# arnauqb/GradABM-JUNE

Measured on NVIDIA B200. Metric: agent_timesteps_per_sec_fwd_bwd, higher is better.
Workload: dtype f32

## Files before the change

### gradabm-june_b200/csrc/gj_kernels.cu

```cuda
#include <cuda_runtime.h>
#include <math.h>
#include <stdint.h>
#include <stdio.h>
#include <stdlib.h>
#include <string.h>

#include "gj_device.cuh"
#include "gj_tiled.cuh"
#include "gj_lean.cuh"
#include "gj_pipe.cuh"

namespace gj {

static thread_local char g_err[512] = "";

static int fail(const char* what, cudaError_t e) {
  snprintf(g_err, sizeof(g_err), "%s: %s", what, cudaGetErrorString(e));
  return -2;
}
static int bad(const char* what) {
  snprintf(g_err, sizeof(g_err), "invalid argument: %s", what);
  return -1;
}
#define GJ_CHECK_LAUNCH(name)                         \
// ... 743 lines not shown
  if (w->n_small > 0 || w->n_chunks > 0) {
    ProfScope ps(bwd ? K_GROUP_CHUNK_B : K_GROUP_CHUNK_F, st);
    const int chunk_blocks = w->n_chunks > 0 ? blocks_for(w->n_chunks * 32, kBlock) : 0;
    const int small_blocks = w->n_small > 0 ? blocks_for(w->n_small, kBlock) : 0;
    launch_pdl(k_lean_group_sums, dim3((chunk_blocks + small_blocks) * bt.nb), dim3(kBlock), 0, st, *w, *p, pl, beta, in,
               out_scaled, out_plain, sc.part_a, chunk_blocks, bt);
    GJ_CHECK_LAUNCH("k_lean_group_sums");
  }
  if (w->n_big > 0) {
    ProfScope ps(bwd ? K_GROUP_FIX_B : K_GROUP_FIX_F, st);
    launch_pdl(k_lean_group_fix, dim3(blocks_for(w->n_big * 32, kBlock) * bt.nb), dim3(kBlock), 0, st, *w, *p, pl, beta,
               (const float*)sc.part_a, out_scaled, out_plain, bt);
    GJ_CHECK_LAUNCH("k_lean_group_fix");
  }
  return 0;
}

static int lean_forward(const gj_world_desc* w, const gj_step_params* p, const Plan& pl, const LeanPlan& lp,
                        const gj_fwd_io* io, const Scratch& sc, cudaStream_t st, const NextStep* next,
                        const Batch& bt = kNoBatch) {
  const bool quar = p->n_quar > 0;
  const bool batch = bt.nb > 1;
  if (p->stage != GJ_STAGE_REST) {
    if (!p->t_ready) {
      ProfScope ps(K_TRANSMISSION, st);
      static OccCache occ[4];
      const Scatter sct{sc.sct_acc, sc.sct_dirty};
#define GJ_K1(Q, B, I)                                                                                               \
  launch_pdl(k_lean_transmission<Q, B>, dim3(lean_grid(w, k_lean_transmission<Q, B>, &occ[I], bt)), dim3(kLeanThreads), \
             0, st, *w, *p, lp, *io, sc.tile_part, sct, bt)
#define GJ_K1C(Q, B, I)                                                                                              \
  launch_pdl(k_lean_transmission_c<Q, B>, dim3(lean_grid(w, k_lean_transmission_c<Q, B>, &occ_c[I], bt)),              \
             dim3(kLeanThreads), 0, st, *w, *p, lp, *io, sc.tile_part, sct, bt)
      static OccCache occ_c[4];
      const bool compact = (pipe_flags() & 4) == 0;
      if (compact) {
        if (batch) {
          if (quar) GJ_K1C(true, true, 3);
          else GJ_K1C(false, true, 2);
        } else {
          if (quar) GJ_K1C(true, false, 1);
          else GJ_K1C(false, false, 0);
        }
      } else if (batch) {
        if (quar) GJ_K1(true, true, 3);
        else GJ_K1(false, true, 2);
      } else {
        if (quar) GJ_K1(true, false, 1);
        else GJ_K1(false, false, 0);
      }
#undef GJ_K1
#undef GJ_K1C
      GJ_CHECK_LAUNCH("k_lean_transmission");
    }
    if (lp.has_generic)
      if (int e = launch_lean_forward_sums(w, p, pl, io->beta, quar ? io->Tq : io->T, io->S_scaled + lp.gen_base,
                                           io->S_unscaled + lp.gen_base, sc, st, bt))
        return e;
    if (int e = launch_cell_groups(w, p, pl, io->beta, io->S_scaled, io->S_unscaled, sc, st, bt)) return e;
  }
  if (p->stage == GJ_STAGE_SUMS) return 0;
  if (int e = launch_cell_gather(w, p, pl, io->S_scaled, sc, st, bt)) return e;
  if (batch && bt.noise && pipe_enabled() && pipe_aligned_fwd(w, lp, io)) {
    ProfScope pn(K_OTHER, st);
    launch_pdl(k_batch_noise, dim3(agent_grid(w->n_agents)), dim3(kBlock), 0, st, *w, *p, const_cast<float*>(bt.noise));
    GJ_CHECK_LAUNCH("k_batch_noise");
  }
  if (pipe_enabled() && pipe_aligned_fwd(w, lp, io)) {
    ProfScope ps(K_AGENT_FWD, st);
    static OccCache occ[20];
    const bool diag = io->q || io->n;
    const bool lab = io->label != nullptr;
    const size_t smem = next ? sizeof(PipeFwdSharedT<true, false>)
                             : (batch ? sizeof(PipeFwdSharedT<false, true>) : sizeof(PipeFwdSharedT<false, false>));
    NextStep nx;
    memset(&nx, 0, sizeof(nx));
    if (next) {
      nx = *next;
      nx.tile_part = sc.tile_part;
      nx.sct = Scatter{sc.sct_acc, sc.sct_dirty};
    }
#define GJ_PIPE_FWD(Q, D, X, B, L, I)                                                                                 \
  launch_pdl(k_pipe_forward<Q, D, X, B, L>,                                                                           \
             dim3(pipe_grid(w, k_pipe_forward<Q, D, X, B, L>, kPipeThreads, smem, &occ[I], bt)), dim3(kPipeThreads),    \
             smem, st, *w, *p, lp, *io, (const float*)sc.cell_buf, sc.red_part, sc.tickets, nx, bt)
    if (lab && batch) {
      if (quar && diag) GJ_PIPE_FWD(true, true, false, true, true, 19);
      else if (quar) GJ_PIPE_FWD(true, false, false, true, true, 18);
      else if (diag) GJ_PIPE_FWD(false, true, false, true, true, 17);
      else GJ_PIPE_FWD(false, false, false, true, true, 16);
    } else if (lab) {
      if (quar && diag) GJ_PIPE_FWD(true, true, false, false, true, 15);
      else if (quar) GJ_PIPE_FWD(true, false, false, false, true, 14);
      else if (diag) GJ_PIPE_FWD(false, true, false, false, true, 13);
      else GJ_PIPE_FWD(false, false, false, false, true, 12);
    } else if (batch) {
      if (quar && diag) GJ_PIPE_FWD(true, true, false, true, false, 11);
      else if (quar) GJ_PIPE_FWD(true, false, false, true, false, 10);
      else if (diag) GJ_PIPE_FWD(false, true, false, true, false, 9);
      else GJ_PIPE_FWD(false, false, false, true, false, 8);
    } else if (next) {
      if (quar && diag) GJ_PIPE_FWD(true, true, true, false, false, 7);
      else if (quar) GJ_PIPE_FWD(true, false, true, false, false, 6);
      else if (diag) GJ_PIPE_FWD(false, true, true, false, false, 5);
      else GJ_PIPE_FWD(false, false, true, false, false, 4);
    } else {
      if (quar && diag) GJ_PIPE_FWD(true, true, false, false, false, 3);
      else if (quar) GJ_PIPE_FWD(true, false, false, false, false, 2);
      else if (diag) GJ_PIPE_FWD(false, true, false, false, false, 1);
      else GJ_PIPE_FWD(false, false, false, false, false, 0);
    }
#undef GJ_PIPE_FWD
    GJ_CHECK_LAUNCH("k_pipe_forward");
    return next ? 1 : 0;
  }
  if (batch) return bad("batched step: the pipelined kernels are off or an array is not 16-byte aligned");
  {
    ProfScope ps(K_AGENT_FWD, st);
    static OccCache occ[8];
    const bool diag = io->q || io->n;
#define GJ_LEAN_FWD(Q, D, L, I)                                                                                       \
  k_lean_forward<Q, D, L><<<lean_grid(w, k_lean_forward<Q, D, L>, &occ[I]), kLeanThreads, 0, st>>>(                   \
      *w, *p, lp, *io, sc.cell_buf, sc.red_part, sc.tickets)
    if (io->label) {
      if (quar && diag) GJ_LEAN_FWD(true, true, true, 7);
      else if (quar) GJ_LEAN_FWD(true, false, true, 6);
      else if (diag) GJ_LEAN_FWD(false, true, true, 5);
      else GJ_LEAN_FWD(false, false, true, 4);
    } else {
      if (quar && diag) GJ_LEAN_FWD(true, true, false, 3);
      else if (quar) GJ_LEAN_FWD(true, false, false, 2);
      else if (diag) GJ_LEAN_FWD(false, true, false, 1);
      else GJ_LEAN_FWD(false, false, false, 0);
    }
#undef GJ_LEAN_FWD
    GJ_CHECK_LAUNCH("k_lean_forward");
  }
  return 0;
}

static int lean_backward(const gj_world_desc* w, const gj_step_params* p, const Plan& pl, LeanPlan lp,
                         const gj_bwd_io* io, const Scratch& sc, cudaStream_t st, const Batch& bt = kNoBatch) {
  const bool quar = p->n_quar > 0;
  const bool batch = bt.nb > 1;
  static OccCache occ_b[4], occ_g[2];
  const bool lab = io->label && io->g_red_label;
  int gather_grid = 1;
  const bool pipe = pipe_enabled() && pipe_aligned_bwd(w, lp, io);
  if (batch && !pipe) return bad("batched step: the pipelined kernels are off or an array is not 16-byte aligned");
  if (p->stage != GJ_STAGE_REST) {
    if (pipe) {
      ProfScope ps(K_AGENT_BWD, st);
      static OccCache occ[8];
      const size_t smem = sizeof(PipeBwdShared);
#define GJ_PIPE_BWD(Q, B, L, I)                                                                                       \
  launch_pdl(k_pipe_backward<Q, B, L>, dim3(pipe_grid(w, k_pipe_backward<Q, B, L>, kBwdThreads, smem, &occ[I], bt)),    \
             dim3(kBwdThreads), smem, st, *w, *p, lp, *io, sc.tile_part, bt)
      if (lab && batch) {
        if (quar) GJ_PIPE_BWD(true, true, true, 7);
        else GJ_PIPE_BWD(false, true, true, 6);
      } else if (lab) {
        if (quar) GJ_PIPE_BWD(true, false, true, 5);
        else GJ_PIPE_BWD(false, false, true, 4);
      } else if (batch) {
        if (quar) GJ_PIPE_BWD(true, true, false, 3);
        else GJ_PIPE_BWD(false, true, false, 2);
      } else {
// ... 767 lines not shown
```

### gradabm-june_b200/csrc/gj_lean.cuh

```cuda
#pragma once
#include "gj_tiled.cuh"

namespace gj {

constexpr int kLeanThreads = 256;
#ifndef GJ_LEAN_MINB_FWD
#define GJ_LEAN_MINB_FWD 3
#endif
#ifndef GJ_LEAN_MINB_BWD
#define GJ_LEAN_MINB_BWD 4
#endif
#ifndef GJ_LEAN_MINB_GATHER
#define GJ_LEAN_MINB_GATHER 3
#endif
constexpr uint32_t kEntNone = 0xFFFFFFFFu;
constexpr uint32_t kEntMulti = 0xFFFFFFFEu;
constexpr uint32_t kEntGiant = 0x80000000u;
constexpr uint32_t kEntId = 0x7FFFFFFFu;

struct Scatter {
  unsigned long long* acc;
  uint8_t* dirty;
};
constexpr float kScatterScale = (float)(1ull << GJ_SCATTER_FRAC);
// ... 57 lines not shown
  const float sg = d + 1e-10f;
  const float sign01 = (sg > 0.0f) ? 1.0f : ((sg == 0.0f) ? 0.5f : 0.0f);
  const float x = d * pf.y;
  const float pe = ex2_fast(fmaf(pf.z, lg2_fast(x), -x * 1.4426950408889634f));
  TransTerms r;
  r.coef = (pf.x * sign01) * pe;
  r.dcoef = 0.0f;
  if (kGrad) r.dcoef = r.coef * pf.y * (1.0f - pf.z * rcp_fast(x));
  return r;
}

__global__ void __launch_bounds__(kBlock) k_profile_pack(int64_t n, const float* __restrict__ maxinf,
                                                         const float* __restrict__ shape,
                                                         const float* __restrict__ rate,
                                                         const float* __restrict__ shift, const float* __restrict__ k0,
                                                         float4* __restrict__ out) {
  const int64_t stride = (int64_t)gridDim.x * blockDim.x;
  for (int64_t a = (int64_t)blockIdx.x * blockDim.x + threadIdx.x; a < n; a += stride)
    out[a] = make_float4((maxinf[a] * k0[a]) * rate[a], rate[a], shape[a] - 1.0f, shift[a]);
}

struct TileRun {
  int64_t t0, t1;
};
__device__ __forceinline__ TileRun lean_tiles(const gj_world_desc& w) {
  TileRun r;
  r.t0 = w.n_tiles * (int64_t)blockIdx.x / gridDim.x;
  r.t1 = w.n_tiles * ((int64_t)blockIdx.x + 1) / gridDim.x;
  return r;
}
__device__ __forceinline__ TileRun lean_tiles(const gj_world_desc& w, const BatchCta& bc) {
  TileRun r;
  r.t0 = w.n_tiles * (int64_t)bc.bx / bc.gx;
  r.t1 = w.n_tiles * ((int64_t)bc.bx + 1) / bc.gx;
  return r;
}
__device__ __forceinline__ int64_t lean_segment_end(const LeanPlan& lp, int64_t tile, int64_t t1) {
  int64_t e = t1;
  for (int i = 0; i < lp.n_tc; ++i) {
    const int64_t c = lp.ctp[i][lp.tc[i][tile] + 1];
    e = c < e ? c : e;
  }
  return e;
}
__device__ __forceinline__ bool lean_new_cell(const LeanPlan& lp, int64_t a, int64_t b) {
  bool changed = false;
  for (int i = 0; i < lp.n_tc; ++i) changed = changed || (lp.tc[i][a] != lp.tc[i][b]);
  return changed;
}

struct alignas(16) ProbRow {
  float v[GJ_MAX_CHANNELS];
};
template <bool kCareSide>
__device__ __forceinline__ void lean_load_prob(ProbRow* prob, const gj_step_params& p, const LeanPlan& lp,
                                               const float* __restrict__ lprob) {
  for (int i = threadIdx.x; i < GJ_MAX_CHANNELS * 200; i += blockDim.x) {
    const int j = i / 200, c = i - j * 200;
    float v = 0.0f;
    if (j < lp.n_cell) {
      v = lprob[(size_t)(lp.c_row[j] * 2 + p.day_type) * 200 + c];
      if (kCareSide && lp.c_care[j] && age_of(c) <= 75) v = 0.0f;
    }
    prob[c].v[j] = v;
  }
}

__device__ __forceinline__ void lean_channel_fma(float (&acc)[GJ_MAX_CHANNELS], const ProbRow* prob, int cls, float x,
                                                 int n_cell) {
  const float4 lo = *reinterpret_cast<const float4*>(&prob[cls].v[0]);
  acc[0] = fmaf(lo.x, x, acc[0]);
  acc[1] = fmaf(lo.y, x, acc[1]);
  acc[2] = fmaf(lo.z, x, acc[2]);
  acc[3] = fmaf(lo.w, x, acc[3]);
  if (n_cell > 4) {
    const float4 hi = *reinterpret_cast<const float4*>(&prob[cls].v[4]);
    acc[4] = fmaf(hi.x, x, acc[4]);
    acc[5] = fmaf(hi.y, x, acc[5]);
    acc[6] = fmaf(hi.z, x, acc[6]);
    acc[7] = fmaf(hi.w, x, acc[7]);
  }
}

__device__ __forceinline__ void lean_class_table(float* __restrict__ L, const ProbRow* prob, const LeanPlan& lp,
                                                 const float* __restrict__ cell_buf, int64_t tile) {
  const int lane = threadIdx.x & 31;
  float mine = 0.0f;
  if (lane < lp.n_cell)
    mine = cell_buf[(lp.c_cell_off[lane] + lp.c_tile_cell[lane][tile]) * GJ_MAX_CHANNELS + lane];
  float acc = 0.0f;
  const int c = threadIdx.x < 200 ? threadIdx.x : 0;
#pragma unroll
  for (int j = 0; j < GJ_MAX_CHANNELS; ++j) {
    const float v = __shfl_sync(0xffffffffu, mine, j);
    acc = fmaf(v, prob[c].v[j], acc);
  }
  if (threadIdx.x < 200) L[threadIdx.x] = acc;
}

__device__ __forceinline__ float lean_generic_issue(const float* __restrict__ buf, uint32_t ent) {
  return (ent < kEntMulti) ? buf[ent & kEntId] : 0.0f;
}
__device__ __forceinline__ float lean_generic_finish(const gj_world_desc& w, const float* __restrict__ buf, uint32_t ent,
                                                     uint32_t a, float v) {
  if (ent == kEntMulti) {
    for (uint32_t j = w.am_ptr[a]; j < w.am_ptr[a + 1]; ++j) {
      const uint32_t e = w.am_ent[j];
      v += buf[w.type_group_off[e >> 28] + (e & 0x0FFFFFFFu)];
    }
  }
  return v;
}

struct RangeLoads {
  float x[8];
};
__device__ __forceinline__ RangeLoads lean_range_issue(const float* __restrict__ v, uint32_t a, uint32_t slot) {
  RangeLoads r;
  const uint32_t b0 = a - (slot >> 16);
  const int nb = (slot == kNoSlot) ? 0 : (int)(slot & 0xFFFFu);
#pragma unroll
  for (int j = 0; j < 8; ++j) r.x[j] = (j < nb) ? v[b0 + j] : 0.0f;
  return r;
}
__device__ __forceinline__ float lean_range_finish(const RangeLoads& r, const float* __restrict__ v, uint32_t a,
                                                   uint32_t slot) {
  float S = ((r.x[0] + r.x[1]) + (r.x[2] + r.x[3])) + ((r.x[4] + r.x[5]) + (r.x[6] + r.x[7]));
  if (slot != kNoSlot && (slot & 0xFFFFu) > 8u) {
    const uint32_t b0 = a - (slot >> 16), nb = slot & 0xFFFFu;
    for (uint32_t b = b0 + 8; b < b0 + nb; ++b) S += v[b];
  }
  return S;
}

__device__ __forceinline__ float quar_mask(const gj_step_params& p, float cur) {
  bool ok = true;
#pragma unroll
  for (int i = 0; i < GJ_MAX_QUAR; ++i)
    if (i < p.n_quar) ok = ok && (cur < p.quar_thr[i]);
  return ok ? 1.0f : 0.0f;
}

#ifndef GJ_K1_BATCH
#define GJ_K1_BATCH 2
#endif
#ifndef GJ_K1_MINB
#define GJ_K1_MINB 7
#endif
constexpr int kK1Batch = GJ_K1_BATCH;

template <bool kQuar, bool kBatch>
__global__ void __launch_bounds__(kLeanThreads, GJ_K1_MINB) k_lean_transmission(gj_world_desc w, gj_step_params p, LeanPlan lp,
                                                                    gj_fwd_io io, float* __restrict__ tile_part,
                                                                    Scatter sct, Batch bt) {
  __shared__ ProbRow prob[200];
  pdl_launch();
  lean_load_prob<false>(prob, p, lp, io.leisure_prob);
  pdl_wait();
  __syncthreads();
  const BatchCta bc = batch_cta<kBatch>(bt);
  const uint32_t so = bc.so;
  if (kBatch) {
    tile_part = scr_shift(tile_part, bt, bc.s);
    sct.acc = scr_shift(sct.acc, bt, bc.s);
    sct.dirty = scr_shift(sct.dirty, bt, bc.s);
  }
  const float4* __restrict__ prof = reinterpret_cast<const float4*>(io.prof4);
  const float* __restrict__ g_inf = io.inf;
  const float* __restrict__ g_cur = io.cur;
  const TileRun run = lean_tiles(w, bc);
  for (int64_t tile = run.t0; tile < run.t1;) {
    const int64_t tend = lp.n_cell > 0 ? lean_segment_end(lp, tile, run.t1) : run.t1;
    const uint32_t a0 = w.tile_begin[tile], a1 = w.tile_begin[tend];
    float acc[GJ_MAX_CHANNELS];
#pragma unroll
    for (int j = 0; j < GJ_MAX_CHANNELS; ++j) acc[j] = 0.0f;
    for (uint32_t base = a0 + threadIdx.x; base < a1; base += kK1Batch * kLeanThreads) {
      float inf[kK1Batch], cur[kK1Batch];
#pragma unroll
// ... 897 lines not shown
```

### gradabm-june_b200/csrc/gj_pipe.cuh

```cuda
#pragma once
#include "gj_lean.cuh"

namespace gj {

constexpr int kPipeThreads = 512;
constexpr int kPipeTile = GJ_TILE_AGENTS;
constexpr int kPipeHalo = 64;
constexpr int kPipeStages = 2;
constexpr int kPipeWarps = kPipeThreads / 32;
constexpr int kPipePer = kPipeTile / kPipeThreads;
static_assert(kPipePer * kPipeThreads == kPipeTile, "tile = whole agents per thread");

__device__ __forceinline__ uint32_t smem_u32(const void* p) { return (uint32_t)__cvta_generic_to_shared(p); }
__device__ __forceinline__ void mbar_init(uint64_t* bar, uint32_t count) {
  asm volatile("mbarrier.init.shared::cta.b64 [%0], %1;" ::"r"(smem_u32(bar)), "r"(count));
}
__device__ __forceinline__ void mbar_expect_tx(uint64_t* bar, uint32_t bytes) {
  asm volatile("mbarrier.arrive.expect_tx.shared::cta.b64 _, [%0], %1;" ::"r"(smem_u32(bar)), "r"(bytes) : "memory");
}
__device__ __forceinline__ void mbar_wait(uint64_t* bar, uint32_t parity) {
  asm volatile(
      "{\n"
      ".reg .pred p;\n"
      "WAIT_%=:\n"
      "mbarrier.try_wait.parity.shared::cta.b64 p, [%0], %1;\n"
      "@p bra DONE_%=;\n"
      "bra WAIT_%=;\n"
      "DONE_%=:\n"
      "}\n" ::"r"(smem_u32(bar)),
      "r"(parity)
      : "memory");
}
__device__ __forceinline__ void bulk_g2s(void* dst, const void* src, uint32_t bytes, uint64_t* bar) {
  asm volatile("cp.async.bulk.shared::cluster.global.mbarrier::complete_tx::bytes [%0], [%1], %2, [%3];" ::"r"(
                   smem_u32(dst)),
               "l"(src), "r"(bytes), "r"(smem_u32(bar))
               : "memory");
}

struct TileSpan {
  uint32_t a0, a1, lo4, hi4, n4;
  uint32_t tlo, thi;
  uint32_t lo16, hi16;
};
__device__ __forceinline__ TileSpan tile_span(const gj_world_desc& w, int64_t tile) {
  TileSpan t;
  t.a0 = w.tile_begin[tile];
  t.a1 = w.tile_begin[tile + 1];
  t.lo4 = t.a0 & ~3u;
  t.hi4 = (t.a1 + 3u) & ~3u;
  t.n4 = (t.hi4 - t.lo4) * 4u;
  const uint32_t nmax = (uint32_t)((w.n_agents + 3) & ~(int64_t)3);
  t.tlo = (t.a0 > (uint32_t)kPipeHalo ? t.a0 - kPipeHalo : 0u) & ~3u;
  t.thi = (t.a1 + kPipeHalo + 3u) & ~3u;
  if (t.thi > nmax) t.thi = nmax;
  t.lo16 = t.a0 & ~15u;
  t.hi16 = (t.a1 + 15u) & ~15u;
  return t;
}
__device__ __forceinline__ uint32_t halo_lo(uint32_t a0) { return (a0 > (uint32_t)kPipeHalo ? a0 - kPipeHalo : 0u) & ~3u; }

struct Copier {
  uint64_t* bar;
  __device__ __forceinline__ void f4(void* dst, const void* base, const TileSpan& t) const {
    bulk_g2s(dst, reinterpret_cast<const char*>(base) + (size_t)t.lo4 * 4u, t.n4, bar);
  }
};

__device__ __forceinline__ float pipe_range_sum(const float* __restrict__ Ts, uint32_t tlo, uint32_t a, uint32_t slot) {
  if (slot == kNoSlot) return 0.0f;
  const uint32_t b0 = a - (slot >> 16) - tlo;
  const int nb = (int)(slot & 0xFFFFu);
  float x[8];
#pragma unroll
  for (int j = 0; j < 8; ++j) x[j] = (j < nb) ? Ts[b0 + j] : 0.0f;
  float S = ((x[0] + x[1]) + (x[2] + x[3])) + ((x[4] + x[5]) + (x[6] + x[7]));
  for (int j = 8; j < nb; ++j) S += Ts[b0 + j];
  return S;
}

struct TileWalk {
  uint32_t a1;
  uint32_t nxt_a1;
  uint32_t nxt_flag;
};
__device__ __forceinline__ TileWalk tile_walk_begin(const gj_world_desc& w, const LeanPlan& lp, const TileRun& run) {
  TileWalk t;
  t.a1 = t.nxt_a1 = 0;
  t.nxt_flag = 1u;
  if (run.t0 < run.t1) {
    t.a1 = w.tile_begin[run.t0];
    t.nxt_a1 = w.tile_begin[run.t0 + 1];
  }
  return t;
}
#define PIPE_TILE_FACTS                                                   \
  const uint32_t a0 = tw.a1, a1 = tw.nxt_a1;                              \
  const bool new_cell = lp.n_cell > 0 && (tw.nxt_flag & 1u);              \
  (void)new_cell;                                                         \
  tw.a1 = a1;                                                             \
  tw.nxt_flag = w.tile_flags[tile + 1];                                   \
  tw.nxt_a1 = w.tile_begin[tile + 2]
#define PIPE_FLUSH(tw, lp) ((lp).n_cell > 0 && (tile + 1 == run.t1 || ((tw).nxt_flag & 1u)))

__device__ __forceinline__ bool pipe_release() {
  __syncthreads();
  return threadIdx.x == 0;
}

constexpr int kPcLut = kPipeHalo + 8;
__device__ __forceinline__ void pipe_fill_pc_lut(float* lut) {
  for (int n = threadIdx.x; n < kPcLut; n += blockDim.x) lut[n] = fmaxf(fminf(1.0f / (float)(n - 1), 1.0f), 0.0f);
}

constexpr int kPipeF = kPipeTile + 8;
constexpr int kPipeH = kPipeTile + 2 * kPipeHalo + 8;

__device__ __forceinline__ void pipe_init_barriers(uint64_t* full) {
  if (threadIdx.x == 0) {
    for (int i = 0; i < kPipeStages; ++i) mbar_init(&full[i], 1);
    asm volatile("fence.mbarrier_init.release.cluster;" ::: "memory");
  }
}

struct NextStep {
  int on;
  float now;
  int day_type;
  int n_quar;
  float quar_thr[GJ_MAX_QUAR];
  int n_cell;
  int c_row[GJ_MAX_CHANNELS];
  int n_tc;
  const uint32_t* tc[GJ_MAX_CHANNELS];
  float* T;
  float* Tq;
  float* tile_part;
  int has_generic;
  Scatter sct;
};
__device__ __forceinline__ float quar_mask_next(const NextStep& nx, float cur) {
  bool ok = true;
#pragma unroll
  for (int i = 0; i < GJ_MAX_QUAR; ++i)
    if (i < nx.n_quar) ok = ok && (cur < nx.quar_thr[i]);
  return ok ? 1.0f : 0.0f;
}
__device__ __forceinline__ bool next_new_cell(const NextStep& nx, int64_t a, int64_t b) {
  bool changed = false;
  for (int i = 0; i < nx.n_tc; ++i) changed = changed || (nx.tc[i][a] != nx.tc[i][b]);
  return changed;
}
template <bool kBatch>
struct alignas(16) PipeFwdStageT {
  float s[kPipeF], inf[kPipeF], tinf[kPipeF], cur[kPipeF], nxt[kPipeF], ttn[kPipeF], rpc[kPipeF];
  uint32_t ent[kPipeF], slot[kPipeF], oid[kPipeF];
  float T[kPipeH];
  uint8_t cls[kPipeTile + 32];
  float dE[kBatch ? kPipeF : 4];
};
template <bool kNext, bool kBatch>
struct PipeFwdSharedT {
  PipeFwdStageT<kBatch> st[kPipeStages];
  ProbRow prob[200];
  ProbRow prob_next[kNext ? 200 : 1];
  float L[2][200];
  float beta[GJ_MAX_NETS];
  float hist[100];
  float deaths;
  float pc_lut[kPcLut];
  alignas(8) uint64_t full[kPipeStages];
};

template <bool kBatch>
__device__ __forceinline__ void pipe_fwd_issue(PipeFwdStageT<kBatch>& sg, uint64_t* bar, const gj_world_desc& w,
                                               const LeanPlan& lp, const gj_fwd_io& io, const float* Tr, int64_t tile,
                                               bool has_gen, bool has_range, uint32_t so = 0u,
                                               const float* noise = nullptr) {
  const TileSpan t = tile_span(w, tile);
  uint32_t total = 6u * t.n4 + (t.hi16 - t.lo16);
  if (kBatch && noise) total += t.n4;
  if (has_gen) total += t.n4;
  if (w.orig_id) total += t.n4;
  if (has_range) total += (lp.r_pc_lut ? 1u : 2u) * t.n4 + (t.thi - t.tlo) * 4u;
  mbar_expect_tx(bar, total);
  const Copier c{bar};
  if (kBatch && noise) c.f4(sg.dE, noise, t);
  if (w.orig_id) c.f4(sg.oid, w.orig_id, t);
  c.f4(sg.s, io.s + so, t);
  c.f4(sg.inf, io.inf + so, t);
  c.f4(sg.tinf, io.tinf + so, t);
  c.f4(sg.cur, io.cur + so, t);
  c.f4(sg.nxt, io.nxt + so, t);
  c.f4(sg.ttn, io.ttn + so, t);
  if (has_gen) c.f4(sg.ent, w.ent1, t);
  if (has_range) {
    c.f4(sg.slot, lp.r_slot, t);
    if (!lp.r_pc_lut) c.f4(sg.rpc, lp.r_pc, t);
    bulk_g2s(sg.T, Tr + so + t.tlo, (t.thi - t.tlo) * 4u, bar);
  }
  bulk_g2s(sg.cls, w.cls + t.lo16, t.hi16 - t.lo16, bar);
}

template <bool kQuar, bool kDiag, bool kNext, bool kBatch, bool kLabel>
__global__ void __launch_bounds__(kPipeThreads, 2) k_pipe_forward(gj_world_desc w, gj_step_params p, LeanPlan lp,
                                                                 gj_fwd_io io, const float* __restrict__ cell_buf,
                                                                 double* __restrict__ red_part,
                                                                 unsigned int* __restrict__ ticket, NextStep nx,
                                                                 Batch bt) {
  static_assert(!(kNext && kBatch), "the look-ahead transmission pass is not batched");
  static_assert(!(kNext && kLabel), "a step with a label table runs without the look-ahead");
  extern __shared__ __align__(128) unsigned char pipe_smem[];
  PipeFwdSharedT<kNext, kBatch>& sh = *reinterpret_cast<PipeFwdSharedT<kNext, kBatch>*>(pipe_smem);
  const BatchCta bc = batch_cta<kBatch>(bt);
  const float* noise = kBatch ? bt.noise : nullptr;
  const uint32_t so = bc.so;
  float* __restrict__ red_out = io.red;
  const float* __restrict__ beta_in = io.beta;
  uint32_t* __restrict__ lacc = io.label_acc;
  if (kBatch) {
    cell_buf = scr_shift(cell_buf, bt, bc.s);
    red_part = scr_shift(red_part, bt, bc.s);
    ticket = scr_shift(ticket, bt, bc.s);
    if (red_out) red_out += (int64_t)bc.s * bt.sRed;
    if (kLabel) lacc += bc.s * bt.sLab;
    beta_in += (int64_t)bc.s * bt.sBeta;
  }
  const TileRun run = lean_tiles(w, bc);
  const float* __restrict__ Tr = (kQuar && !lp.r_house) ? io.Tq : io.T;
  const bool has_gen = lp.has_generic != 0, has_range = lp.n_range > 0;
  pdl_launch();
  pipe_init_barriers(sh.full);
  lean_load_prob<true>(sh.prob, p, lp, io.leisure_prob);
  pipe_fill_pc_lut(sh.pc_lut);
  if (kNext) {
    for (int i = threadIdx.x; i < GJ_MAX_CHANNELS * 200; i += blockDim.x) {
      const int j = i / 200, c = i - j * 200;
      sh.prob_next[c].v[j] = j < nx.n_cell ? io.leisure_prob[(size_t)(nx.c_row[j] * 2 + nx.day_type) * 200 + c] : 0.0f;
    }
  }
  pdl_wait();
  if (threadIdx.x < p.n_nets) sh.beta[threadIdx.x] = beta_in[threadIdx.x];
  if (threadIdx.x < 100) sh.hist[threadIdx.x] = 0.0f;
  if (threadIdx.x == 0) sh.deaths = 0.0f;
  __syncthreads();
  if (threadIdx.x == 0) {
    for (int i = 0; i < kPipeStages; ++i)
      if (run.t0 + i < run.t1)
        pipe_fwd_issue<kBatch>(sh.st[i], &sh.full[i], w, lp, io, Tr, run.t0 + i, has_gen, has_range, so, noise);
  }
  const float* __restrict__ SP = io.S_scaled + lp.gen_base + (kBatch ? (int64_t)bc.s * bt.sG : (int64_t)0);
  const float dead = (float)(p.n_stages - 1);
  const float inv_tau = 1.0f / p.tau;
  const float beta_r = lp.n_range > 0 ? sh.beta[lp.r_net] : 0.0f;

  const float4* __restrict__ prof = reinterpret_cast<const float4*>(io.prof4);
  float acc[GJ_MAX_CHANNELS];
#pragma unroll
  for (int j = 0; j < GJ_MAX_CHANNELS; ++j) acc[j] = 0.0f;
  int nbuild = 0, stg = 0;
  uint32_t parity = 0;
  const float* L = sh.L[0];
  TileWalk tw = tile_walk_begin(w, lp, run);
  for (int64_t tile = run.t0; tile < run.t1; ++tile) {
    PipeFwdStageT<kBatch>& sg = sh.st[stg];
    PIPE_TILE_FACTS;
    mbar_wait(&sh.full[stg], parity);
    if (new_cell) {
      lean_class_table(sh.L[nbuild & 1], sh.prob, lp, cell_buf, tile);
      L = sh.L[nbuild & 1];
      ++nbuild;
      __syncthreads();
    }
    const uint32_t sk = a0 & 3u, sk16 = a0 & 15u, tlo = halo_lo(a0);
    uint32_t ent[kPipePer];
    float gen[kPipePer];
    float4 pfe[kPipePer];
#pragma unroll
    for (int h = 0; h < kPipePer; ++h) {
      const uint32_t j = threadIdx.x + h * kPipeThreads;
      ent[h] = (has_gen && a0 + j < a1) ? sg.ent[j + sk] : kEntNone;
      gen[h] = lean_generic_issue(SP, ent[h]);
      if (kNext) {
        pfe[h] = make_float4(0.0f, 0.0f, 0.0f, 0.0f);
        if (a0 + j < a1 && sg.inf[j + sk] != 0.0f) pfe[h] = prof[a0 + j];
      }
    }
#pragma unroll
    for (int h = 0; h < kPipePer; ++h) {
      const uint32_t j = threadIdx.x + h * kPipeThreads;
      const uint32_t a = a0 + j, i = j + sk;
      if (a >= a1) break;
      const float hs = has_range ? pipe_range_sum(sg.T, tlo, a, sg.slot[i]) : 0.0f;
      const int cls = sg.cls[j + sk16];
      const float Lc = lp.n_cell > 0 ? L[cls] : 0.0f;
      const float gv = lean_generic_finish(w, SP, ent[h], a, gen[h]);
      const uint64_t ga = w.orig_id ? (uint64_t)sg.oid[i] : p.agent_offset + a;
      const float rpc = !has_range ? 0.0f : (lp.r_pc_lut ? ((sg.slot[i] == kNoSlot) ? 0.0f : sh.pc_lut[sg.slot[i] & 0xFFFFu])
                                                         : sg.rpc[i]);
      const FwdOut o = lean_forward_agent<kQuar, kDiag>(p, lp, io, a + so, ga, hs, gv, Lc, beta_r, rpc,
                                                        sg.s[i], sg.inf[i], sg.tinf[i], sg.cur[i], sg.nxt[i], sg.ttn[i], cls,
                                                        inv_tau, dead, sh.hist, &sh.deaths, kBatch && noise != nullptr,
                                                        (kBatch && noise) ? sg.dE[i] : 0.0f);
      if (kLabel) label_add(lacc, io.label, a, (uint32_t)o.inf, o.cur == dead ? 1u : 0u);
      if (kNext) {
        float T = 0.0f;
        if (o.inf != 0.0f) {
          const float4 pf = (sg.inf[i] != 0.0f) ? pfe[h] : prof[a];
          T = lean_transmission<false>(nx.now, o.tinf, pf).coef * o.inf;
        }
        nx.T[a] = T;
        float Tq = T;
        if (nx.n_quar > 0) {
          Tq = quar_mask_next(nx, o.cur) * T;
          nx.Tq[a] = Tq;
        }
        if (Tq != 0.0f) {
          if (nx.n_cell > 0) lean_channel_fma(acc, sh.prob_next, cls, Tq, nx.n_cell);
          if (nx.has_generic) lean_scatter(w, nx.sct, has_gen ? ent[h] : w.ent1[a], a, Tq);
        }
      }
    }
    if (pipe_release() && tile + kPipeStages < run.t1)
      pipe_fwd_issue<kBatch>(sg, &sh.full[stg], w, lp, io, Tr, tile + kPipeStages, has_gen, has_range, so, noise);
    if (++stg == kPipeStages) {
      stg = 0;
      parity ^= 1u;
    }
    if (kNext && nx.n_cell > 0) {
      if (tile + 1 == run.t1 || next_new_cell(nx, tile, tile + 1)) {
        block_sums<float, GJ_MAX_CHANNELS, kPipeWarps>(acc, nx.n_cell, nx.tile_part + tile * GJ_MAX_CHANNELS);
#pragma unroll
        for (int j = 0; j < GJ_MAX_CHANNELS; ++j) acc[j] = 0.0f;
      } else if ((int)threadIdx.x < nx.n_cell) {
        nx.tile_part[tile * GJ_MAX_CHANNELS + threadIdx.x] = 0.0f;
      }
    }
  }
  if (red_out) {
    __syncthreads();
    const int nr = 2 + p.n_age_bins;
    if ((int)threadIdx.x < nr) {
      double v = 0.0;
      if (threadIdx.x == 0) {
        for (int c = 0; c < 100; ++c) v += (double)sh.hist[c];
      } else if (threadIdx.x == 1) {
        v = (double)sh.deaths;
      } else {
        const int b = threadIdx.x - 2;
        for (int c = max(p.age_bins[b] + 1, 0); c < p.age_bins[b + 1] && c < 100; ++c) v += (double)sh.hist[c];
      }
      red_part[(int64_t)bc.bx * kMaxRed + threadIdx.x] = v;
    }
    finish_partials<kMaxRed>(nr, red_part, bc.gx, ticket, red_out);
  }
}

struct alignas(16) PipeBwdStage {
  float s[kPipeF], tinf[kPipeF], cur[kPipeF], nxt[kPipeF], ttn[kPipeF], ty[kPipeF], v[kPipeF];
  uint8_t cls[kPipeTile + 32];
};
struct PipeBwdShared {
  PipeBwdStage st[kPipeStages];
  ProbRow prob[200];
  float gred_age[100];
  uint32_t next_flag[kPipeStages];
  alignas(8) uint64_t full[kPipeStages];
};
struct BwdCot {
  const float* p[6];
};

__device__ __forceinline__ void pipe_bwd_issue(PipeBwdStage& sg, uint64_t* bar, const gj_world_desc& w,
                                               const gj_bwd_io& io, int64_t tile, uint32_t so = 0u) {
  const TileSpan t = tile_span(w, tile);
  const uint32_t total = 7u * t.n4 + (t.hi16 - t.lo16);
  mbar_expect_tx(bar, total);
  const Copier c{bar};
  c.f4(sg.s, io.s + so, t);
  c.f4(sg.tinf, io.tinf + so, t);
  c.f4(sg.cur, io.cur + so, t);
  c.f4(sg.nxt, io.nxt + so, t);
  c.f4(sg.ttn, io.ttn + so, t);
  c.f4(sg.ty, io.tape_y0 + so, t);
  c.f4(sg.v, io.tape_v + so, t);
  bulk_g2s(sg.cls, w.cls + t.lo16, t.hi16 - t.lo16, bar);
}

#ifndef GJ_PIPE_BWD_THREADS
#define GJ_PIPE_BWD_THREADS 512
#endif
constexpr int kBwdThreads = GJ_PIPE_BWD_THREADS;
constexpr int kBwdPer = kPipeTile / kBwdThreads;
constexpr int kBwdCtas = kBwdThreads == 256 ? 3 : 2;
template <bool kQuar, bool kBatch, bool kLabel>
__global__ void __launch_bounds__(kBwdThreads, kBwdCtas) k_pipe_backward(gj_world_desc w, gj_step_params p, LeanPlan lp,
                                                                  gj_bwd_io io, float* __restrict__ tile_part,
                                                                  Batch bt) {
  extern __shared__ __align__(128) unsigned char pipe_smem[];
  PipeBwdShared& sh = *reinterpret_cast<PipeBwdShared*>(pipe_smem);
  const BatchCta bc = batch_cta<kBatch>(bt);
  const uint32_t so = bc.so;
  const float* __restrict__ g_red = io.g_red;
  const float* __restrict__ g_lab = io.g_red_label;
  if (kBatch) {
    tile_part = scr_shift(tile_part, bt, bc.s);
    if (g_red) g_red += (int64_t)bc.s * bt.sRed;
    if (kLabel) g_lab += bc.s * bt.sLab;
  }
  const TileRun run = lean_tiles(w, bc);
  const BwdCot cot{{io.g_s_o, io.g_inf_o, io.g_tinf_o, io.g_cur_o, io.g_nxt_o, io.g_ttn_o}};
  pdl_launch();
  pipe_init_barriers(sh.full);
  lean_load_prob<true>(sh.prob, p, lp, io.leisure_prob);
  pdl_wait();
  if (threadIdx.x < 100) {
    float g = 0.0f;
    if (g_red) {
// ... 202 lines not shown
```

### gradabm-june_b200/csrc/gj_tiled.cuh

```cuda
#pragma once
#include "gj_device.cuh"

namespace gj {

constexpr uint32_t kNoSlot = 0xFFFFFFFFu;

struct Plan {
  int n_t2;
  int t2_net[GJ_MAX_CHANNELS];
  int net_t2[GJ_MAX_NETS];
  int n_t1;
  int t1_net[GJ_MAX_RANGE_NETS];
  int net_t1[GJ_MAX_NETS];
  int n_lei;
  int lei_net[GJ_MAX_CHANNELS];
  int net_lei[GJ_MAX_NETS];
  int n_generic;
  int tier[GJ_MAX_NETS];
  const uint32_t* slot[GJ_MAX_NETS];
  const float* rpc[GJ_MAX_NETS];
};

struct Batch {
  int nb;
  uint32_t sN;
  int64_t sG;
  int64_t sScr;
  int sBeta, sRed;
  const float* noise;
  int64_t sLab;
};
struct BatchCta {
  int s;
  uint32_t bx, gx;
  uint32_t so;
};
template <bool kBatch>
__device__ __forceinline__ BatchCta batch_cta(const Batch& bt) {
  BatchCta c;
  if (kBatch) {
    c.s = (int)(blockIdx.x % (uint32_t)bt.nb);
    c.bx = blockIdx.x / (uint32_t)bt.nb;
    c.gx = gridDim.x / (uint32_t)bt.nb;
    c.so = (uint32_t)c.s * bt.sN;
  } else {
    c.s = 0;
    c.bx = blockIdx.x;
    c.gx = gridDim.x;
    c.so = 0u;
  }
  return c;
}
template <typename T>
__device__ __forceinline__ T* scr_shift(T* p, const Batch& bt, int s) {
  return reinterpret_cast<T*>(reinterpret_cast<char*>(p) + (int64_t)s * bt.sScr);
}
template <typename T>
__device__ __forceinline__ const T* scr_shift(const T* p, const Batch& bt, int s) {
  return reinterpret_cast<const T*>(reinterpret_cast<const char*>(p) + (int64_t)s * bt.sScr);
}

struct TileTables {
  float prob[GJ_MAX_CHANNELS][200];
  float beta[GJ_MAX_NETS];
  float cellv[GJ_MAX_CHANNELS];
};

__device__ __forceinline__ void load_tables(TileTables& tb, const gj_step_params& p, const Plan& pl,
                                            const float* __restrict__ lprob, const float* __restrict__ beta) {
  for (int i = threadIdx.x; i < pl.n_lei * 200; i += blockDim.x) {
    const int j = i / 200, c = i - j * 200;
    tb.prob[j][c] = lprob[(size_t)(p.nets[pl.lei_net[j]].prob_row * 2 + p.day_type) * 200 + c];
  }
  if (threadIdx.x < p.n_nets) tb.beta[threadIdx.x] = beta ? beta[threadIdx.x] : 0.0f;
}

__device__ __forceinline__ void load_cell_values(TileTables& tb, const gj_world_desc& w, const gj_step_params& p,
                                                 const Plan& pl, const float* __restrict__ cell_buf, int64_t tile) {
  if (threadIdx.x < pl.n_t2) {
    const int t = p.nets[pl.t2_net[threadIdx.x]].type;
    const uint32_t cell = w.tile_cell[t][tile];
    tb.cellv[threadIdx.x] = cell_buf[(w.cell_off[t] + cell) * GJ_MAX_CHANNELS + threadIdx.x];
  }
}

__device__ __forceinline__ float member_value(const TileTables& tb, const Plan& pl, int k, int kind, float v0, float v1,
                                              int cls) {
  if (kind == GJ_KIND_HOUSEHOLD) return v0;
  if (kind == GJ_KIND_PLAIN) return v1;
  return tb.prob[pl.net_lei[k]][cls] * v1;
}

template <typename T, int kR, int kWarps = kBlock / 32>
__device__ __forceinline__ void block_sums(T (&v)[kR], int nr, T* __restrict__ out ) {
  __shared__ T sm[kWarps][kR];
  const int lane = threadIdx.x & 31, wid = threadIdx.x >> 5;
#pragma unroll
  for (int r = 0; r < kR; ++r)
    if (r < nr) v[r] = warp_sum(v[r]);
  if (lane == 0) {
#pragma unroll
    for (int r = 0; r < kR; ++r)
      if (r < nr) sm[wid][r] = v[r];
  }
  __syncthreads();
  if (threadIdx.x < nr) {
    T s = (T)0;
#pragma unroll
    for (int k = 0; k < kWarps; ++k) s += sm[k][threadIdx.x];
    out[threadIdx.x] = s;
  }
  __syncthreads();
}

template <int kR>
__device__ __forceinline__ void finish_partials(int nr, const double* __restrict__ partials, int64_t n_part,
                                                unsigned int* __restrict__ ticket, float* __restrict__ out) {
  __shared__ bool last;
  __shared__ double sm[32];
  __threadfence();
  __syncthreads();
  if (threadIdx.x == 0) last = (atomicAdd(ticket, 1u) == (unsigned int)n_part - 1u);
  __syncthreads();
  if (!last) return;
  __threadfence();
  for (int r = 0; r < nr; ++r) {
    double s = 0.0;
    for (int64_t b = threadIdx.x; b < n_part; b += blockDim.x) s += partials[b * kR + r];
    s = warp_sum(s);
    if ((threadIdx.x & 31) == 0) sm[threadIdx.x >> 5] = s;
    __syncthreads();
    if (threadIdx.x == 0) {
      double tsum = 0.0;
      for (int k = 0; k < (int)(blockDim.x / 32); ++k) tsum += sm[k];
      out[r] = (float)tsum;
    }
    __syncthreads();
  }
  if (threadIdx.x == 0) *ticket = 0u;
}

__global__ void __launch_bounds__(kBlock) k_tile_transmission(gj_world_desc w, gj_step_params p, Plan pl, gj_fwd_io io,
                                                              float* __restrict__ tile_part) {
  __shared__ TileTables tb;
  const int64_t tile = blockIdx.x;
  const uint32_t a0 = w.tile_begin[tile], a1 = w.tile_begin[tile + 1];
  if (pl.n_t2 > 0) load_tables(tb, p, pl, io.leisure_prob, nullptr);
  __syncthreads();
  float acc[GJ_MAX_CHANNELS];
#pragma unroll
  for (int j = 0; j < GJ_MAX_CHANNELS; ++j) acc[j] = 0.0f;
  const bool quar = p.n_quar > 0;
  for (uint32_t a = a0 + threadIdx.x; a < a1; a += kBlock) {
    float T = 0.0f;
    if (io.T_in) {
      T = io.T_in[a];
    } else {
      const float inf = io.inf[a];
      if (inf != 0.0f) {
        const TransTerms tt =
            transmission_terms<false>(p.now, io.tinf[a], io.maxinf[a], io.shape[a], io.rate[a], io.shift[a], io.k0[a]);
        T = tt.coef * inf;
      }
      io.T[a] = T;
    }
    float Tq = T;
    if (quar) {
      Tq = quarantine_mask(p, io.cur[a]) * T;
      io.Tq[a] = Tq;
    }
    if (pl.n_t2 > 0 && T != 0.0f) {
      const int cls = w.cls[a];
#pragma unroll
      for (int j = 0; j < GJ_MAX_CHANNELS; ++j)
        if (j < pl.n_t2) acc[j] += member_value(tb, pl, pl.t2_net[j], p.nets[pl.t2_net[j]].kind, T, Tq, cls);
    }
  }
  if (pl.n_t2 > 0) block_sums<float, GJ_MAX_CHANNELS>(acc, pl.n_t2, tile_part + tile * GJ_MAX_CHANNELS);
}

__global__ void __launch_bounds__(kBlock) k_cell_groups(gj_world_desc w, gj_step_params p, Plan pl,
                                                        const float* __restrict__ beta,
                                                        const float* __restrict__ tile_part,
                                                        float* __restrict__ out_scaled, float* __restrict__ out_plain,
                                                        Batch bt) {
  pdl_launch();
  pdl_wait();
  if (bt.nb > 1) {
    const int s = blockIdx.z;
    beta += (int64_t)s * bt.sBeta;
    tile_part = scr_shift(tile_part, bt, s);
    out_scaled += (int64_t)s * bt.sG;
    out_plain += (int64_t)s * bt.sG;
  }
  const int j = blockIdx.y;
// ... 497 lines not shown
```

Baseline: 21.15 billion.

## Add producer warps to forward pipe kernel for gather and class-table prefetch

Result: slower. 18.48 billion (median of 6 runs) (-12.6%).

```diff
diff --git a/gradabm-june_b200/csrc/gj_kernels.cu b/gradabm-june_b200/csrc/gj_kernels.cu
--- a/gradabm-june_b200/csrc/gj_kernels.cu
+++ b/gradabm-june_b200/csrc/gj_kernels.cu
@@ -849,7 +849,8 @@
     }
 #define GJ_PIPE_FWD(Q, D, X, B, L, I)                                                                                 \
   launch_pdl(k_pipe_forward<Q, D, X, B, L>,                                                                           \
-             dim3(pipe_grid(w, k_pipe_forward<Q, D, X, B, L>, kPipeThreads, smem, &occ[I], bt)), dim3(kPipeThreads),    \
+             dim3(pipe_grid(w, k_pipe_forward<Q, D, X, B, L>, kPipeFwdThreads, smem, &occ[I], bt)),                   \
+             dim3(kPipeFwdThreads),                                                                                   \
              smem, st, *w, *p, lp, *io, (const float*)sc.cell_buf, sc.red_part, sc.tickets, nx, bt)
     if (lab && batch) {
       if (quar && diag) GJ_PIPE_FWD(true, true, false, true, true, 19);
diff --git a/gradabm-june_b200/csrc/gj_lean.cuh b/gradabm-june_b200/csrc/gj_lean.cuh
--- a/gradabm-june_b200/csrc/gj_lean.cuh
+++ b/gradabm-june_b200/csrc/gj_lean.cuh
@@ -163,19 +163,26 @@
   }
 }
 
-__device__ __forceinline__ void lean_class_table(float* __restrict__ L, const ProbRow* prob, const LeanPlan& lp,
-                                                 const float* __restrict__ cell_buf, int64_t tile) {
+__device__ __forceinline__ float lean_cell_value(const LeanPlan& lp, const float* __restrict__ cell_buf, int64_t tile) {
   const int lane = threadIdx.x & 31;
   float mine = 0.0f;
   if (lane < lp.n_cell)
     mine = cell_buf[(lp.c_cell_off[lane] + lp.c_tile_cell[lane][tile]) * GJ_MAX_CHANNELS + lane];
+  return mine;
+}
+__device__ __forceinline__ float lean_class_value(const ProbRow* prob, int c, float mine) {
   float acc = 0.0f;
-  const int c = threadIdx.x < 200 ? threadIdx.x : 0;
 #pragma unroll
   for (int j = 0; j < GJ_MAX_CHANNELS; ++j) {
     const float v = __shfl_sync(0xffffffffu, mine, j);
     acc = fmaf(v, prob[c].v[j], acc);
   }
+  return acc;
+}
+__device__ __forceinline__ void lean_class_table(float* __restrict__ L, const ProbRow* prob, const LeanPlan& lp,
+                                                 const float* __restrict__ cell_buf, int64_t tile) {
+  const float mine = lean_cell_value(lp, cell_buf, tile);
+  const float acc = lean_class_value(prob, threadIdx.x < 200 ? threadIdx.x : 0, mine);
   if (threadIdx.x < 200) L[threadIdx.x] = acc;
 }
 
diff --git a/gradabm-june_b200/csrc/gj_pipe.cuh b/gradabm-june_b200/csrc/gj_pipe.cuh
--- a/gradabm-june_b200/csrc/gj_pipe.cuh
+++ b/gradabm-june_b200/csrc/gj_pipe.cuh
@@ -17,6 +17,9 @@
 }
 __device__ __forceinline__ void mbar_expect_tx(uint64_t* bar, uint32_t bytes) {
   asm volatile("mbarrier.arrive.expect_tx.shared::cta.b64 _, [%0], %1;" ::"r"(smem_u32(bar)), "r"(bytes) : "memory");
+}
+__device__ __forceinline__ void mbar_arrive(uint64_t* bar) {
+  asm volatile("mbarrier.arrive.shared::cta.b64 _, [%0];" ::"r"(smem_u32(bar)) : "memory");
 }
 __device__ __forceinline__ void mbar_wait(uint64_t* bar, uint32_t parity) {
   asm volatile(
@@ -151,36 +154,41 @@
   for (int i = 0; i < nx.n_tc; ++i) changed = changed || (nx.tc[i][a] != nx.tc[i][b]);
   return changed;
 }
+constexpr int kPipeProducers = 2;
+constexpr int kPipeFwdThreads = kPipeThreads + 32 * kPipeProducers;
+constexpr int kPipeFwdVals = kPipeTile / (32 * kPipeProducers);
 template <bool kBatch>
 struct alignas(16) PipeFwdStageT {
   float s[kPipeF], inf[kPipeF], tinf[kPipeF], cur[kPipeF], nxt[kPipeF], ttn[kPipeF], rpc[kPipeF];
-  uint32_t ent[kPipeF], slot[kPipeF], oid[kPipeF];
+  uint32_t slot[kPipeF], oid[kPipeF];
   float T[kPipeH];
   uint8_t cls[kPipeTile + 32];
   float dE[kBatch ? kPipeF : 4];
+  float gv[kPipeTile];
+  float L[200];
+  uint32_t a0, a1;
 };
 template <bool kNext, bool kBatch>
 struct PipeFwdSharedT {
   PipeFwdStageT<kBatch> st[kPipeStages];
   ProbRow prob[200];
   ProbRow prob_next[kNext ? 200 : 1];
-  float L[2][200];
   float beta[GJ_MAX_NETS];
   float hist[100];
   float deaths;
   float pc_lut[kPcLut];
   alignas(8) uint64_t full[kPipeStages];
+  uint64_t ready[kPipeStages];
+  uint64_t empty[kPipeStages];
 };
 
 template <bool kBatch>
 __device__ __forceinline__ void pipe_fwd_issue(PipeFwdStageT<kBatch>& sg, uint64_t* bar, const gj_world_desc& w,
-                                               const LeanPlan& lp, const gj_fwd_io& io, const float* Tr, int64_t tile,
-                                               bool has_gen, bool has_range, uint32_t so = 0u,
+                                               const LeanPlan& lp, const gj_fwd_io& io, const float* Tr,
+                                               const TileSpan& t, bool has_range, uint32_t so = 0u,
                                                const float* noise = nullptr) {
-  const TileSpan t = tile_span(w, tile);
   uint32_t total = 6u * t.n4 + (t.hi16 - t.lo16);
   if (kBatch && noise) total += t.n4;
-  if (has_gen) total += t.n4;
   if (w.orig_id) total += t.n4;
   if (has_range) total += (lp.r_pc_lut ? 1u : 2u) * t.n4 + (t.thi - t.tlo) * 4u;
   mbar_expect_tx(bar, total);
@@ -193,7 +201,6 @@
   c.f4(sg.cur, io.cur + so, t);
   c.f4(sg.nxt, io.nxt + so, t);
   c.f4(sg.ttn, io.ttn + so, t);
-  if (has_gen) c.f4(sg.ent, w.ent1, t);
   if (has_range) {
     c.f4(sg.slot, lp.r_slot, t);
     if (!lp.r_pc_lut) c.f4(sg.rpc, lp.r_pc, t);
@@ -202,8 +209,86 @@
   bulk_g2s(sg.cls, w.cls + t.lo16, t.hi16 - t.lo16, bar);
 }
 
+__device__ __forceinline__ void pipe_fwd_gather(float (&v)[kPipeFwdVals], const gj_world_desc& w,
+                                                const float* __restrict__ SP, const TileSpan& t, uint32_t pt) {
+  const uint32_t n = t.a1 - t.a0;
+  uint32_t e[kPipeFwdVals];
+#pragma unroll
+  for (int k = 0; k < kPipeFwdVals; ++k) {
+    const uint32_t j = pt + 32u * kPipeProducers * k;
+    e[k] = __ldg(&w.ent1[t.a0 + (j < n ? j : 0u)]);
+  }
+  uint32_t multi = 0;
+#pragma unroll
+  for (int k = 0; k < kPipeFwdVals; ++k) {
+    const uint32_t j = pt + 32u * kPipeProducers * k;
+    const uint32_t ek = j < n ? e[k] : kEntNone;
+    const float x = __ldg(&SP[ek < kEntMulti ? (ek & kEntId) : 0u]);
+    v[k] = ek < kEntMulti ? x : 0.0f;
+    multi |= (ek == kEntMulti ? 1u : 0u) << k;
+  }
+#pragma unroll
+  for (int k = 0; k < kPipeFwdVals; ++k)
+    if (multi & (1u << k)) v[k] = lean_generic_finish(w, SP, kEntMulti, t.a0 + pt + 32u * kPipeProducers * k, v[k]);
+}
+
+template <bool kNext, bool kBatch>
+__device__ __forceinline__ void pipe_fwd_produce(PipeFwdSharedT<kNext, kBatch>& sh, const TileRun& run,
+                                                 const gj_world_desc& w, const LeanPlan& lp, const gj_fwd_io& io,
+                                                 const float* Tr, const float* __restrict__ SP,
+                                                 const float* __restrict__ cell_buf, bool has_gen, bool has_range,
+                                                 uint32_t so, const float* noise) {
+  const uint32_t pt = threadIdx.x - kPipeThreads;
+  uint32_t parity = 0, cell = 0, held[kPipeStages] = {~0u, ~0u};
+  int stg = 0;
+  float v[kPipeFwdVals];
+  TileSpan t{};
+  if (run.t0 < run.t1) {
+    t = tile_span(w, run.t0);
+    if (has_gen) pipe_fwd_gather(v, w, SP, t, pt);
+  }
+  for (int64_t tile = run.t0; tile < run.t1; ++tile) {
+    PipeFwdStageT<kBatch>& sg = sh.st[stg];
+    if (tile >= run.t0 + kPipeStages) mbar_wait(&sh.empty[stg], parity ^ 1u);
+    if (pt == 0) {
+      sg.a0 = t.a0;
+      sg.a1 = t.a1;
+      pipe_fwd_issue<kBatch>(sg, &sh.full[stg], w, lp, io, Tr, t, has_range, so, noise);
+    }
+    if (has_gen) {
+#pragma unroll
+      for (int k = 0; k < kPipeFwdVals; ++k) {
+        const uint32_t j = pt + 32u * kPipeProducers * k;
+        if (j < t.a1 - t.a0) sg.gv[j] = v[k];
+      }
+    }
+    if (lp.n_cell > 0) {
+      if (tile == run.t0 || (w.tile_flags[tile] & 1u)) ++cell;
+      if ((stg ? held[1] : held[0]) != cell) {
+        const float mine = lean_cell_value(lp, cell_buf, tile);
+        for (uint32_t c0 = 0; c0 < 200u; c0 += 32u * kPipeProducers) {
+          const uint32_t c = c0 + pt;
+          const float x = lean_class_value(sh.prob, c < 200u ? (int)c : 0, mine);
+          if (c < 200u) sg.L[c] = x;
+        }
+        if (stg) held[1] = cell;
+        else held[0] = cell;
+      }
+    }
+    mbar_arrive(&sh.ready[stg]);
+    if (++stg == kPipeStages) {
+      stg = 0;
+      parity ^= 1u;
+    }
+    if (tile + 1 < run.t1) {
+      t = tile_span(w, tile + 1);
+      if (has_gen) pipe_fwd_gather(v, w, SP, t, pt);
+    }
+  }
+}
+
 template <bool kQuar, bool kDiag, bool kNext, bool kBatch, bool kLabel>
-__global__ void __launch_bounds__(kPipeThreads, 2) k_pipe_forward(gj_world_desc w, gj_step_params p, LeanPlan lp,
+__global__ void __launch_bounds__(kPipeFwdThreads, 2) k_pipe_forward(gj_world_desc w, gj_step_params p, LeanPlan lp,
                                                                  gj_fwd_io io, const float* __restrict__ cell_buf,
                                                                  double* __restrict__ red_part,
                                                                  unsigned int* __restrict__ ticket, NextStep nx,
@@ -230,7 +315,14 @@
   const float* __restrict__ Tr = (kQuar && !lp.r_house) ? io.Tq : io.T;
   const bool has_gen = lp.has_generic != 0, has_range = lp.n_range > 0;
   pdl_launch();
-  pipe_init_barriers(sh.full);
+  if (threadIdx.x == 0) {
+    for (int i = 0; i < kPipeStages; ++i) {
+      mbar_init(&sh.full[i], 1);
+      mbar_init(&sh.ready[i], 32 * kPipeProducers);
+      mbar_init(&sh.empty[i], kPipeWarps);
+    }
+    asm volatile("fence.mbarrier_init.release.cluster;" ::: "memory");
+  }
   lean_load_prob<true>(sh.prob, p, lp, io.leisure_prob);
   pipe_fill_pc_lut(sh.pc_lut);
   if (kNext) {
@@ -244,96 +336,84 @@
   if (threadIdx.x < 100) sh.hist[threadIdx.x] = 0.0f;
   if (threadIdx.x == 0) sh.deaths = 0.0f;
   __syncthreads();
-  if (threadIdx.x == 0) {
-    for (int i = 0; i < kPipeStages; ++i)
-      if (run.t0 + i < run.t1)
-        pipe_fwd_issue<kBatch>(sh.st[i], &sh.full[i], w, lp, io, Tr, run.t0 + i, has_gen, has_range, so, noise);
-  }
   const float* __restrict__ SP = io.S_scaled + lp.gen_base + (kBatch ? (int64_t)bc.s * bt.sG : (int64_t)0);
-  const float dead = (float)(p.n_stages - 1);
-  const float inv_tau = 1.0f / p.tau;
-  const float beta_r = lp.n_range > 0 ? sh.beta[lp.r_net] : 0.0f;
-
-  const float4* __restrict__ prof = reinterpret_cast<const float4*>(io.prof4);
-  float acc[GJ_MAX_CHANNELS];
-#pragma unroll
-  for (int j = 0; j < GJ_MAX_CHANNELS; ++j) acc[j] = 0.0f;
-  int nbuild = 0, stg = 0;
-  uint32_t parity = 0;
-  const float* L = sh.L[0];
-  TileWalk tw = tile_walk_begin(w, lp, run);
-  for (int64_t tile = run.t0; tile < run.t1; ++tile) {
-    PipeFwdStageT<kBatch>& sg = sh.st[stg];
-    PIPE_TILE_FACTS;
-    mbar_wait(&sh.full[stg], parity);
-    if (new_cell) {
-      lean_class_table(sh.L[nbuild & 1], sh.prob, lp, cell_buf, tile);
-      L = sh.L[nbuild & 1];
-      ++nbuild;
-      __syncthreads();
-    }
-    const uint32_t sk = a0 & 3u, sk16 = a0 & 15u, tlo = halo_lo(a0);
-    uint32_t ent[kPipePer];
-    float gen[kPipePer];
-    float4 pfe[kPipePer];
-#pragma unroll
-    for (int h = 0; h < kPipePer; ++h) {
-      const uint32_t j = threadIdx.x + h * kPipeThreads;
-      ent[h] = (has_gen && a0 + j < a1) ? sg.ent[j + sk] : kEntNone;
-      gen[h] = lean_generic_issue(SP, ent[h]);
+  if (threadIdx.x >= kPipeThreads) {
+    pipe_fwd_produce<kNext, kBatch>(sh, run, w, lp, io, Tr, SP, cell_buf, has_gen, has_range, so, noise);
+  } else {
+    const float dead = (float)(p.n_stages - 1);
+    const float inv_tau = 1.0f / p.tau;
+    const float beta_r = lp.n_range > 0 ? sh.beta[lp.r_net] : 0.0f;
+
+    const float4* __restrict__ prof = reinterpret_cast<const float4*>(io.prof4);
+    float acc[GJ_MAX_CHANNELS];
+#pragma unroll
+    for (int j = 0; j < GJ_MAX_CHANNELS; ++j) acc[j] = 0.0f;
+    int stg = 0;
+    uint32_t parity = 0;
+    for (int64_t tile = run.t0; tile < run.t1; ++tile) {
+      PipeFwdStageT<kBatch>& sg = sh.st[stg];
+      mbar_wait(&sh.full[stg], parity);
+      mbar_wait(&sh.ready[stg], parity);
+      const uint32_t a0 = sg.a0, a1 = sg.a1;
+      const uint32_t sk = a0 & 3u, sk16 = a0 & 15u, tlo = halo_lo(a0);
+      float4 pfe[kPipePer];
       if (kNext) {
-        pfe[h] = make_float4(0.0f, 0.0f, 0.0f, 0.0f);
-        if (a0 + j < a1 && sg.inf[j + sk] != 0.0f) pfe[h] = prof[a0 + j];
-      }
-    }
-#pragma unroll
-    for (int h = 0; h < kPipePer; ++h) {
-      const uint32_t j = threadIdx.x + h * kPipeThreads;
-      const uint32_t a = a0 + j, i = j + sk;
-      if (a >= a1) break;
-      const float hs = has_range ? pipe_range_sum(sg.T, tlo, a, sg.slot[i]) : 0.0f;
-      const int cls = sg.cls[j + sk16];
-      const float Lc = lp.n_cell > 0 ? L[cls] : 0.0f;
-      const float gv = lean_generic_finish(w, SP, ent[h], a, gen[h]);
-      const uint64_t ga = w.orig_id ? (uint64_t)sg.oid[i] : p.agent_offset + a;
-      const float rpc = !has_range ? 0.0f : (lp.r_pc_lut ? ((sg.slot[i] == kNoSlot) ? 0.0f : sh.pc_lut[sg.slot[i] & 0xFFFFu])
-                                                         : sg.rpc[i]);
-      const FwdOut o = lean_forward_agent<kQuar, kDiag>(p, lp, io, a + so, ga, hs, gv, Lc, beta_r, rpc,
-                                                        sg.s[i], sg.inf[i], sg.tinf[i], sg.cur[i], sg.nxt[i], sg.ttn[i], cls,
-                                                        inv_tau, dead, sh.hist, &sh.deaths, kBatch && noise != nullptr,
-                                                        (kBatch && noise) ? sg.dE[i] : 0.0f);
-      if (kLabel) label_add(lacc, io.label, a, (uint32_t)o.inf, o.cur == dead ? 1u : 0u);
-      if (kNext) {
-        float T = 0.0f;
-        if (o.inf != 0.0f) {
-          const float4 pf = (sg.inf[i] != 0.0f) ? pfe[h] : prof[a];
-          T = lean_transmission<false>(nx.now, o.tinf, pf).coef * o.inf;
-        }
-        nx.T[a] = T;
-        float Tq = T;
-        if (nx.n_quar > 0) {
-          Tq = quar_mask_next(nx, o.cur) * T;
-          nx.Tq[a] = Tq;
-        }
-        if (Tq != 0.0f) {
-          if (nx.n_cell > 0) lean_channel_fma(acc, sh.prob_next, cls, Tq, nx.n_cell);
-          if (nx.has_generic) lean_scatter(w, nx.sct, has_gen ? ent[h] : w.ent1[a], a, Tq);
+#pragma unroll
+        for (int h = 0; h < kPipePer; ++h) {
+          const uint32_t j = threadIdx.x + h * kPipeThreads;
+          pfe[h] = make_float4(0.0f, 0.0f, 0.0f, 0.0f);
+          if (a0 + j < a1 && sg.inf[j + sk] != 0.0f) pfe[h] = prof[a0 + j];
         }
       }
-    }
-    if (pipe_release() && tile + kPipeStages < run.t1)
-      pipe_fwd_issue<kBatch>(sg, &sh.full[stg], w, lp, io, Tr, tile + kPipeStages, has_gen, has_range, so, noise);
-    if (++stg == kPipeStages) {
-      stg = 0;
-      parity ^= 1u;
-    }
-    if (kNext && nx.n_cell > 0) {
-      if (tile + 1 == run.t1 || next_new_cell(nx, tile, tile + 1)) {
-        block_sums<float, GJ_MAX_CHANNELS, kPipeWarps>(acc, nx.n_cell, nx.tile_part + tile * GJ_MAX_CHANNELS);
-#pragma unroll
-        for (int j = 0; j < GJ_MAX_CHANNELS; ++j) acc[j] = 0.0f;
-      } else if ((int)threadIdx.x < nx.n_cell) {
-        nx.tile_part[tile * GJ_MAX_CHANNELS + threadIdx.x] = 0.0f;
+#pragma unroll
+      for (int h = 0; h < kPipePer; ++h) {
+        const uint32_t j = threadIdx.x + h * kPipeThreads;
+        const uint32_t a = a0 + j, i = j + sk;
+        if (a >= a1) break;
+        const float hs = has_range ? pipe_range_sum(sg.T, tlo, a, sg.slot[i]) : 0.0f;
+        const int cls = sg.cls[j + sk16];
+        const float Lc = lp.n_cell > 0 ? sg.L[cls] : 0.0f;
+        const float gv = has_gen ? sg.gv[j] : 0.0f;
+        const uint64_t ga = w.orig_id ? (uint64_t)sg.oid[i] : p.agent_offset + a;
+        const float rpc = !has_range ? 0.0f : (lp.r_pc_lut ? ((sg.slot[i] == kNoSlot) ? 0.0f : sh.pc_lut[sg.slot[i] & 0xFFFFu])
+                                                           : sg.rpc[i]);
+        const FwdOut o = lean_forward_agent<kQuar, kDiag>(p, lp, io, a + so, ga, hs, gv, Lc, beta_r, rpc,
+                                                          sg.s[i], sg.inf[i], sg.tinf[i], sg.cur[i], sg.nxt[i], sg.ttn[i], cls,
+                                                          inv_tau, dead, sh.hist, &sh.deaths, kBatch && noise != nullptr,
+                                                          (kBatch && noise) ? sg.dE[i] : 0.0f);
+        if (kLabel) label_add(lacc, io.label, a, (uint32_t)o.inf, o.cur == dead ? 1u : 0u);
+        if (kNext) {
+          float T = 0.0f;
+          if (o.inf != 0.0f) {
+            const float4 pf = (sg.inf[i] != 0.0f) ? pfe[h] : prof[a];
+            T = lean_transmission<false>(nx.now, o.tinf, pf).coef * o.inf;
+          }
+          nx.T[a] = T;
+          float Tq = T;
+          if (nx.n_quar > 0) {
+            Tq = quar_mask_next(nx, o.cur) * T;
+            nx.Tq[a] = Tq;
+          }
+          if (Tq != 0.0f) {
+            if (nx.n_cell > 0) lean_channel_fma(acc, sh.prob_next, cls, Tq, nx.n_cell);
+            if (nx.has_generic) lean_scatter(w, nx.sct, w.ent1[a], a, Tq);
+          }
+        }
+      }
+      __syncwarp();
+      if ((threadIdx.x & 31u) == 0) mbar_arrive(&sh.empty[stg]);
+      if (++stg == kPipeStages) {
+        stg = 0;
+        parity ^= 1u;
+      }
+      if (kNext && nx.n_cell > 0) {
+        if (tile + 1 == run.t1 || next_new_cell(nx, tile, tile + 1)) {
+          block_sums<float, GJ_MAX_CHANNELS, kPipeWarps, 1>(acc, nx.n_cell, nx.tile_part + tile * GJ_MAX_CHANNELS);
+#pragma unroll
+          for (int j = 0; j < GJ_MAX_CHANNELS; ++j) acc[j] = 0.0f;
+        } else if ((int)threadIdx.x < nx.n_cell) {
+          nx.tile_part[tile * GJ_MAX_CHANNELS + threadIdx.x] = 0.0f;
+        }
       }
     }
   }
diff --git a/gradabm-june_b200/csrc/gj_tiled.cuh b/gradabm-june_b200/csrc/gj_tiled.cuh
--- a/gradabm-june_b200/csrc/gj_tiled.cuh
+++ b/gradabm-june_b200/csrc/gj_tiled.cuh
@@ -91,7 +91,13 @@
   return tb.prob[pl.net_lei[k]][cls] * v1;
 }
 
-template <typename T, int kR, int kWarps = kBlock / 32>
+template <int kBar, int kThreads>
+__device__ __forceinline__ void cta_sync() {
+  if (kBar == 0) __syncthreads();
+  else asm volatile("bar.sync %0, %1;" ::"n"(kBar), "n"(kThreads) : "memory");
+}
+
+template <typename T, int kR, int kWarps = kBlock / 32, int kBar = 0>
 __device__ __forceinline__ void block_sums(T (&v)[kR], int nr, T* __restrict__ out ) {
   __shared__ T sm[kWarps][kR];
   const int lane = threadIdx.x & 31, wid = threadIdx.x >> 5;
@@ -103,14 +109,14 @@
     for (int r = 0; r < kR; ++r)
       if (r < nr) sm[wid][r] = v[r];
   }
-  __syncthreads();
+  cta_sync<kBar, kWarps * 32>();
   if (threadIdx.x < nr) {
     T s = (T)0;
 #pragma unroll
     for (int k = 0; k < kWarps; ++k) s += sm[k][threadIdx.x];
     out[threadIdx.x] = s;
   }
-  __syncthreads();
+  cta_sync<kBar, kWarps * 32>();
 }
 
 template <int kR>
```
